# thangvubk/SoftGroup

Hardware: AMD Instinct MI355X
Metric: scans/sec ScanNet-v2-like inference (softgroup_scannet.yaml, full forward_test) (higher is better)
Workload: dtype f32

## Files before the change

### softgroup_amd/csrc/spconv_conv.hip

```cpp
#include <stdlib.h>

#include <atomic>
#include <cstdio>
#include <map>
#include <mutex>
#include <utility>
#include <vector>

#include "common.h"

namespace sg {

typedef float f32x16 __attribute__((ext_vector_type(16)));
typedef float f4 __attribute__((ext_vector_type(4)));
typedef float f2 __attribute__((ext_vector_type(2)));
typedef __bf16 bf16x8 __attribute__((ext_vector_type(8)));
typedef __bf16 bf16x2 __attribute__((ext_vector_type(2)));

__device__ __forceinline__ void split3(const float (&x)[8], bf16x8 &h, bf16x8 &m, bf16x8 &l) {
#pragma unroll
  for (int j = 0; j < 4; ++j) {
    const f2 v = {x[2 * j], x[2 * j + 1]};
    const bf16x2 hh = __builtin_convertvector(v, bf16x2);
    const f2 r = v - __builtin_convertvector(hh, f2);
// ... 173 lines not shown
    int k2 = k, s2 = s + 1;
    if (s2 == n_slices) {
      s2 = 0;
      const uint32_t rest = mask & ~((2u << k) - 1u);
      k2 = rest ? __builtin_ctz(rest) : -1;
    }
    if (k2 >= 0) load_raw(k2, s2, a_nxt, b_nxt);
    __builtin_amdgcn_sched_barrier(0);
#pragma unroll
    for (int j = 0; j < 8; ++j)
#pragma unroll
      for (int n = 0; n < NBW; ++n)
        acc[n] = __builtin_amdgcn_mfma_f32_32x32x2f32(a_cur[j], b_cur[n][j], acc[n], 0, 0, 0);
    __builtin_amdgcn_sched_barrier(0);
    k = k2;
    s = s2;
  }

  const bool final_out = p.ksplit == 1;
  float *out = p.out + (final_out ? 0 : static_cast<long long>(ks) * p.M_out * p.Cout);
  const bool add_res = p.residual != nullptr && final_out;
  const bool post = p.post_scale != nullptr && final_out;
  const bool act = p.out_act != nullptr && final_out;
  float ps[NBW], pb[NBW], as[NBW], ab[NBW];
#pragma unroll
  for (int n = 0; n < NBW; ++n) {
    ps[n] = post ? p.post_scale[coff[n]] : 1.f;
    pb[n] = post ? p.post_shift[coff[n]] : 0.f;
    as[n] = act ? p.act_scale[coff[n]] : 1.f;
    ab[n] = act ? p.act_shift[coff[n]] : 0.f;
  }
#pragma unroll
  for (int reg = 0; reg < 16; ++reg) {
    const int r = (reg & 3) + 8 * (reg >> 2) + 4 * ahalf;
    const int row = __shfl(my_row, r, 64);
    if (row < 0) continue;
    const long long off = static_cast<long long>(row) * p.Cout + col;
#pragma unroll
    for (int n = 0; n < NBW; ++n) {
      if (n < nbw && col + n * 32 < p.Cout) {
        float v = acc[n][reg];
        if (add_res) v += p.residual[off + n * 32];
        if (post) v = fmaxf(fmaf(v, ps[n], pb[n]), 0.f);
        out[off + n * 32] = v;
        if (act) p.out_act[off + n * 32] = fmaxf(fmaf(v, as[n], ab[n]), 0.f);
      }
    }
  }
}

constexpr int kRowsAt = kTileRows * kMaxK, kMaskAt = kRowsAt + kTileRows;
constexpr int kMetaInts = kMaskAt + 4;

template <int CK, int DEPTH, int TRACE, int NBW, int SPLIT, int WV, int AT, int CHAIN, int R16 = 0>
__device__ __forceinline__ void conv_layer_body(const ConvArgs &p, unsigned in_bytes, unsigned w_bytes) {
  static_assert(!R16 || (SPLIT == 2 && AT), "bf16 rows: bf16-operand arithmetic, line-wise gather");
  constexpr int AUX = CHAIN ? 16 : 0;
  static_assert(!SPLIT || CK == 16 || AT, "split-precision path: 16-channel slices");
  static_assert(!AT || (SPLIT && CK == 32), "line-wise gather: split path, 32-channel items");
  static_assert(WV == 2 || WV == 4 || WV == 8 || WV == 16, "2, 4, 8 or 16 waves per workgroup");
  constexpr int RR = 16 / WV;
  constexpr int WV_SHIFT = WV == 2 ? 1 : WV == 4 ? 2 : WV == 8 ? 3 : 4;
  constexpr int HC = CK / 2;
  constexpr int NQ = HC / 4;
  extern __shared__ __attribute__((aligned(16))) char smem_raw[];
  const int wave = __builtin_amdgcn_readfirstlane(threadIdx.x >> 6), lane = threadIdx.x & 63;
  const int arow = lane & 31, ahalf = lane >> 5;
  float *red = reinterpret_cast<float *>(smem_raw);
  int32_t *meta_lds = reinterpret_cast<int32_t *>(red + WV * NBW * 16 * 64);

  const int G = gridDim.x;
  const int units_per_tile = p.col_units * p.ksplit;
  const int num_units = p.num_units;
  const int n_slices = R16 ? (p.Cin + 63) / 64 : p.Cin / CK;
  const int c8 = p.Cin / 8;
  const int tileK = kTileRows * p.K;
  const int nbr_base = arow * p.K;
  const bool final_out = p.ksplit == 1;
  const bool add_res = p.residual != nullptr && final_out;
  const bool post = p.post_scale != nullptr && final_out;
  const bool act = p.out_act != nullptr && final_out;
  const bool combine = p.done != nullptr && !final_out;
  const int num_tiles = (p.M_out + kTileRows - 1) / kTileRows;
  const unsigned out_bytes = static_cast<unsigned>(p.M_out) * p.Cout * 4u;
  const bool out16 = SPLIT == 2 && p.out16 != 0, res16 = SPLIT == 2 && p.res16 != 0;
  const unsigned fin_bytes = out16 ? out_bytes >> 1 : out_bytes;
  const unsigned res_bytes = res16 ? out_bytes >> 1 : out_bytes;

  const __amdgpu_buffer_rsrc_t rs_in =
      __builtin_amdgcn_make_buffer_rsrc(const_cast<float *>(p.in), 0, in_bytes, 0x00020000);
  const __amdgpu_buffer_rsrc_t rs_w =
      __builtin_amdgcn_make_buffer_rsrc(const_cast<float *>(p.w), 0, w_bytes, 0x00020000);
  const __amdgpu_buffer_rsrc_t rs_res = __builtin_amdgcn_make_buffer_rsrc(
      const_cast<float *>(add_res ? p.residual : p.in), 0, add_res ? res_bytes : 0u, 0x00020000);
  const __amdgpu_buffer_rsrc_t rs_out = __builtin_amdgcn_make_buffer_rsrc(
      p.out, 0, final_out ? fin_bytes : out_bytes * static_cast<unsigned>(p.ksplit), 0x00020000);
  const __amdgpu_buffer_rsrc_t rs_act = __builtin_amdgcn_make_buffer_rsrc(
      act ? p.out_act : p.out, 0, act ? fin_bytes : 0u, 0x00020000);
  const bool c_res = combine && p.residual != nullptr, c_act = combine && p.out_act != nullptr;
  const __amdgpu_buffer_rsrc_t rs_cres = __builtin_amdgcn_make_buffer_rsrc(
      const_cast<float *>(c_res ? p.residual : p.in), 0, c_res ? res_bytes : 0u, 0x00020000);
  const __amdgpu_buffer_rsrc_t rs_cout = __builtin_amdgcn_make_buffer_rsrc(
      combine ? p.out_final : p.out, 0, combine ? fin_bytes : 0u, 0x00020000);
  const __amdgpu_buffer_rsrc_t rs_cact = __builtin_amdgcn_make_buffer_rsrc(
      c_act ? p.out_act : p.out, 0, c_act ? fin_bytes : 0u, 0x00020000);
  auto ld_row = [&](const __amdgpu_buffer_rsrc_t &rs, unsigned off, int n, bool h16) -> float {
    if constexpr (SPLIT == 2) {
      if (h16)
        return bf16_f32(static_cast<uint16_t>(__builtin_amdgcn_raw_buffer_load_b16(rs, off >> 1, n * 64, AUX)));
// ... 19 lines not shown
    Unit d;
    int sub;
    if (u < full) {
      const int blk = udiv(u >> 3, p.magic_upt);
      const int i = u - blk * group;
      d.tile = blk * 8 + (i & 7);
      sub = i >> 3;
    } else {
      d.tile = udiv(u, p.magic_upt);
      sub = u - d.tile * units_per_tile;
    }
    d.ks = udiv(sub, p.magic_cu);
    d.cu = sub - d.ks * p.col_units;
    return d;
  };

  int32_t *ctl = meta_lds + 2 * kMetaInts;
  const unsigned meta_lds_addr = __builtin_amdgcn_readfirstlane(
      static_cast<unsigned>(reinterpret_cast<uintptr_t>(meta_lds)));
  auto dma_meta = [&](int tile, int buf) {
    const unsigned dst = meta_lds_addr + static_cast<unsigned>(buf * kMetaInts) * 4u;
    const int32_t *blk = p.nbr_tiles + static_cast<long long>(tile) * tileK;
#pragma unroll
    for (int q = 0; q < 4; ++q) {
      const int e = q * 256 + lane * 4;
      if (e < tileK) lds_dma_b128(blk + e, dst + q * 1024);
    }
    if (lane < kTileRows) lds_dma_b32(p.order + tile * kTileRows + lane, dst + kRowsAt * 4);
    if (lane == 0) lds_dma_b32(p.tile_mask + tile, dst + kMaskAt * 4);
  };
  (void)num_tiles;

  constexpr int NPL = SPLIT == 2 ? 1 : 3;
  constexpr int NB_ = R16 ? 4 : AT ? 2 * NPL : SPLIT ? NPL : NQ;
  struct Slice { f4 a[NQ]; f4 b[NBW][NB_]; int nsl; };
  const int plane_bytes = p.K * c8 * p.Cout * 16;
  const int planes_at = 2 * plane_bytes;
  struct Ctx {
    const int32_t *meta;
    uint32_t wg_mask;
    int col, ks, k, s, kp, sp, rem;
    int pair;
    int v_w;
    float ps[NBW], pb[NBW], as[NBW], ab[NBW];
    unsigned o_off[RR];
    bool col_ok;
  };

  Slice S[DEPTH];
  float resv[NBW][RR];

  f4 *tr_lds = reinterpret_cast<f4 *>(ctl + 4) + wave * 256;
  const unsigned row_pitch = static_cast<unsigned>(p.Cin) * 4u, lane_chunk = static_cast<unsigned>(lane & 7) * 16u;
  auto load = [&](const Ctx &c, int k, int s, Slice &S) {
    if constexpr (R16) {
#pragma unroll
      for (int q = 0; q < 4; ++q) {
        const unsigned src = static_cast<unsigned>(c.meta[(8 * q + (lane >> 3)) * p.K + k]);
        const unsigned v_a = __umul24(src, row_pitch >> 1) + lane_chunk;
        S.a[q] = __builtin_bit_cast(f4, __builtin_amdgcn_raw_buffer_load_b128(rs_in, v_a, s * 128, AUX));
      }
      const int s_w = planes_at + (k * c8 + s * 8) * p.Cout * 16;
      const int nsl = s * 64 + 64 <= p.Cin ? 4 : 2;
      S.nsl = nsl;
#pragma unroll
      for (int n = 0; n < NBW; ++n)
#pragma unroll
        for (int sl = 0; sl < 4; ++sl)
          S.b[n][sl] = __builtin_bit_cast(f4, __builtin_amdgcn_raw_buffer_load_b128(
                                                  rs_w, c.v_w + n * 512, s_w + (sl < nsl ? sl : sl - 2) * (2 * p.Cout * 16), 0));
      return;
    }
    if constexpr (AT) {
#pragma unroll
      for (int q = 0; q < 4; ++q) {
        unsigned src = static_cast<unsigned>(c.meta[(8 * q + (lane >> 3)) * p.K + k]);
        if (SG_WHATIF & 16) src = static_cast<unsigned>(c.pair * 32 + 8 * q + (lane >> 3)) % static_cast<unsigned>(p.M_out);
        const unsigned v_a = __umul24(src, row_pitch) + lane_chunk;
        S.a[q] = __builtin_bit_cast(f4, __builtin_amdgcn_raw_buffer_load_b128(rs_in, v_a, s * 128, AUX));
      }
      const int s_w = planes_at + (k * c8 + s * 4) * p.Cout * 16;
#pragma unroll
      for (int n = 0; n < NBW; ++n)
#pragma unroll
        for (int sl = 0; sl < 2; ++sl)
#pragma unroll
          for (int pl = 0; pl < NPL; ++pl) {
            if ((SG_WHATIF & 1) && pl > 0) { S.b[n][sl * NPL + pl] = S.b[n][sl * NPL]; continue; }
            S.b[n][sl * NPL + pl] = __builtin_bit_cast(f4, __builtin_amdgcn_raw_buffer_load_b128(
                                                             rs_w, c.v_w + n * 512,
                                                             s_w + sl * (2 * p.Cout * 16) + pl * plane_bytes, 0));
          }
      return;
    }
    const int src = c.meta[nbr_base + k];
    const unsigned v_a = src >= 0 ? static_cast<unsigned>(src * p.Cin + ahalf * HC) * 4u : kOob;
    const int s_a = s * (CK * 4);
#pragma unroll
    for (int q = 0; q < NQ; ++q)
      S.a[q] = __builtin_bit_cast(f4, __builtin_amdgcn_raw_buffer_load_b128(rs_in, v_a + q * 16, s_a, AUX));
    if constexpr (SPLIT) {
      const int s_w = planes_at + (k * c8 + s * 2) * p.Cout * 16;
#pragma unroll
      for (int n = 0; n < NBW; ++n)
#pragma unroll
        for (int pl = 0; pl < NPL; ++pl)
          S.b[n][pl] = __builtin_bit_cast(f4, __builtin_amdgcn_raw_buffer_load_b128(
                                                  rs_w, c.v_w + n * 512, s_w + pl * plane_bytes, 0));
    } else {
      const int s_w = (k * c8 + s * (CK / 8)) * p.Cout * 32;
#pragma unroll
      for (int n = 0; n < NBW; ++n)
#pragma unroll
        for (int q = 0; q < NQ; ++q)
          S.b[n][q] = __builtin_bit_cast(f4, __builtin_amdgcn_raw_buffer_load_b128(
                                                 rs_w, c.v_w + n * 1024 + (q & 1) * 16,
                                                 s_w + (q >> 1) * (p.Cout * 32), 0));
    }
  };

  auto advance = [&](const Ctx &c, int &k, int &s) {
    if (++s == n_slices) {
      s = 0;
      const uint32_t rest = c.wg_mask & ~((2u << k) - 1u);
      k = rest ? __builtin_ctz(rest) : k;
    }
  };

  auto setup = [&](const Unit &d, int buf, Ctx &c) {
    c.ks = d.ks;
    c.pair = d.tile * p.col_units + d.cu;
    c.meta = meta_lds + buf * kMetaInts;
    uint32_t m = static_cast<uint32_t>(c.meta[kMaskAt]);
    if (!final_out) {
      const int k_lo = d.ks * p.k_per_split, k_hi = min(p.K, k_lo + p.k_per_split);
      m &= ((1u << k_hi) - 1u) & ~((1u << k_lo) - 1u);
    }
    m = __builtin_amdgcn_readfirstlane(m);
    c.wg_mask = m;
    c.col = d.cu * (32 * NBW) + arow;
    c.col_ok = c.col < p.Cout;
    const int colc = min(c.col, p.Cout - 1);
    c.v_w = SPLIT ? (ahalf * p.Cout + colc) * 16 : (ahalf * (HC / 8) * p.Cout + colc) * 32;
    const int items = __builtin_popcount(m) * n_slices;
    const int per = (items + WV - 1) >> WV_SHIFT;
// ... 110 lines not shown
          }
          acc[n] = __builtin_amdgcn_mfma_f32_32x32x16_bf16(al, bh, acc[n], 0, 0, 0);
          acc[n] = __builtin_amdgcn_mfma_f32_32x32x16_bf16(am, bm, acc[n], 0, 0, 0);
          acc[n] = __builtin_amdgcn_mfma_f32_32x32x16_bf16(ah, bl, acc[n], 0, 0, 0);
          acc[n] = __builtin_amdgcn_mfma_f32_32x32x16_bf16(am, bh, acc[n], 0, 0, 0);
          acc[n] = __builtin_amdgcn_mfma_f32_32x32x16_bf16(ah, bm, acc[n], 0, 0, 0);
          acc[n] = __builtin_amdgcn_mfma_f32_32x32x16_bf16(ah, bh, acc[n], 0, 0, 0);
        }
      }
      return;
    }
    if constexpr (SPLIT) {
      const float af[8] = {S.a[0][0], S.a[0][1], S.a[0][2], S.a[0][3], S.a[1][0], S.a[1][1], S.a[1][2], S.a[1][3]};
      if constexpr (SPLIT == 2) {
        const bf16x8 ah = round_bf16(af);
#pragma unroll
        for (int n = 0; n < NBW; ++n)
          acc[n] = __builtin_amdgcn_mfma_f32_32x32x16_bf16(ah, __builtin_bit_cast(bf16x8, S.b[n][0]), acc[n], 0,
                                                           0, 0);
        return;
      }
      bf16x8 ah, am, al;
      split3(af, ah, am, al);
#pragma unroll
      for (int n = 0; n < NBW; ++n) {
        const bf16x8 bh = __builtin_bit_cast(bf16x8, S.b[n][0]);
        const bf16x8 bm = __builtin_bit_cast(bf16x8, S.b[n][1]);
        const bf16x8 bl = __builtin_bit_cast(bf16x8, S.b[n][2]);
        acc[n] = __builtin_amdgcn_mfma_f32_32x32x16_bf16(al, bh, acc[n], 0, 0, 0);
        acc[n] = __builtin_amdgcn_mfma_f32_32x32x16_bf16(am, bm, acc[n], 0, 0, 0);
        acc[n] = __builtin_amdgcn_mfma_f32_32x32x16_bf16(ah, bl, acc[n], 0, 0, 0);
        acc[n] = __builtin_amdgcn_mfma_f32_32x32x16_bf16(am, bh, acc[n], 0, 0, 0);
        acc[n] = __builtin_amdgcn_mfma_f32_32x32x16_bf16(ah, bm, acc[n], 0, 0, 0);
        acc[n] = __builtin_amdgcn_mfma_f32_32x32x16_bf16(ah, bh, acc[n], 0, 0, 0);
      }
      return;
    }
#pragma unroll
    for (int q = 0; q < NQ; ++q) {
      asm volatile("" : "+v"(S.a[q]));
#pragma unroll
      for (int n = 0; n < NBW; ++n) asm volatile("" : "+v"(S.b[n][q]));
    }
    __builtin_amdgcn_sched_barrier(0);
#pragma unroll
    for (int q = 0; q < NQ; ++q)
#pragma unroll
      for (int j = 0; j < 4; ++j)
#pragma unroll
        for (int n = 0; n < NBW; ++n)
          acc[n] = __builtin_amdgcn_mfma_f32_32x32x2f32(S.a[q][j], S.b[n][q][j], acc[n], 0, 0, 0);
  };

  unsigned long long stamp[8];
  auto mark = [&](int i) {
    if constexpr (TRACE) stamp[i] = __builtin_readcyclecounter();
  };

  const int xcd = blockIdx.x & 7;
  const int dyn0 = (p.dyn_rounds == 1 ? 1 : 2) * G;
  const bool draws = p.queue != nullptr && dyn0 < num_units;
  const bool draw_first = draws && p.dyn_rounds == 1;
  auto barrier = [] {
    asm volatile("s_waitcnt lgkmcnt(0)\n\ts_barrier" ::: "memory");
  };

  if (static_cast<int>(blockIdx.x) >= num_units) return;
  int round = 0, u = blockIdx.x, buf = 0;
  Unit du = decode(u);
  unsigned ticket = 0;
  bool drawing = true;
  if (wave == 0) {
    if (lane == 0 && draw_first)
      ticket = __hip_atomic_fetch_add(p.queue + xcd * kTicketStride, 1u, __ATOMIC_RELAXED, __HIP_MEMORY_SCOPE_AGENT);
    dma_meta(du.tile, 0);
    asm volatile("s_waitcnt vmcnt(0)" ::: "memory");
  }
  barrier();
  Ctx c;
  setup(du, 0, c);

  while (true) {
    mark(0);
    int un_w0 = -1;
    if (wave == 0) {
      if ((round == 0 && !draw_first) || !draws) {
        const int r = round + 1;
        const int b = static_cast<int>(blockIdx.x);
        const int rev = (G & 7) == 0 ? G - 8 - (b & ~7) + (b & 7) : G - 1 - b;
        un_w0 = r * G + ((__builtin_popcount(r) & 1) ? rev : b);
      } else if (drawing) {
        const unsigned t = __builtin_amdgcn_readfirstlane(ticket);
        un_w0 = dyn0 + static_cast<int>(t) * 8 + xcd;
      }
      if (un_w0 >= num_units || un_w0 < 0) {
        un_w0 = -1;
        drawing = false;
      }
      if (un_w0 >= 0) dma_meta(decode(un_w0).tile, buf ^ 1);
      if (lane == 0) ctl[buf ^ 1] = un_w0;
    }
#pragma unroll
    for (int n = 0; n < NBW; ++n)
#pragma unroll
      for (int r = 0; r < 16; ++r) acc[n][r] = 0.f;
    {
      int kp = c.kp, sp = c.sp, issued = DEPTH - 1;
      const int rem = c.rem;
      for (int g = rem / DEPTH; g > 0; --g) {
#pragma unroll
        for (int i = 0; i < DEPTH; ++i) {
          int k2 = kp, s2 = sp;
          advance(c, k2, s2);
          const bool more = issued < rem;
          kp = more ? k2 : kp;
          sp = more ? s2 : sp;
          ++issued;
          load(c, kp, sp, S[(i + DEPTH - 1) % DEPTH]);
          __builtin_amdgcn_sched_barrier(0);
          compute(S[i]);
          __builtin_amdgcn_sched_barrier(0);
        }
      }
      const int tail = rem % DEPTH;
#pragma unroll
      for (int i = 0; i < DEPTH - 1; ++i)
        if (i < tail) compute(S[i]);
    }
    if constexpr (TRACE) { asm volatile("" : "+v"(acc[0][0])); }
    mark(1);

    if (wave == 0) {
      asm volatile("s_waitcnt vmcnt(0)" ::: "memory");
      if (lane == 0 && draws)
        ticket = __hip_atomic_fetch_add(p.queue + xcd * kTicketStride, 1u, __ATOMIC_RELAXED,
                                        __HIP_MEMORY_SCOPE_AGENT);
    }

    barrier();
    mark(2);
#pragma unroll
    for (int n = 0; n < NBW; ++n)
#pragma unroll
      for (int reg = 0; reg < 16; ++reg) red[((wave * NBW + n) * 16 + reg) * 64 + lane] = acc[n][reg];
    barrier();
    mark(3);
    const int un = __builtin_amdgcn_readfirstlane(ctl[buf ^ 1]);
    const bool has_next = un >= 0;
    const Unit dn = decode(has_next ? un : u);

    float v[NBW][RR], va[NBW][RR];
    unsigned o_off[RR];
    {
      float part[NBW][RR][WV];
#pragma unroll
      for (int n = 0; n < NBW; ++n)
#pragma unroll
        for (int rr = 0; rr < RR; ++rr) {
          const int reg = wave * RR + rr;
// ... 79 lines not shown
          for (int j = 0; j < 4; ++j)
#pragma unroll
            for (int rr = 0; rr < RR; ++rr)
#pragma unroll
              for (int n = 0; n < NBW; ++n) t[n][rr] += q[j][n][rr];
        }
        for (; ks < p.ksplit; ++ks) {
          float q[NBW][RR];
#pragma unroll
          for (int rr = 0; rr < RR; ++rr)
#pragma unroll
            for (int n = 0; n < NBW; ++n) q[n][rr] = part(ks, rr, n);
#pragma unroll
          for (int rr = 0; rr < RR; ++rr)
#pragma unroll
            for (int n = 0; n < NBW; ++n) t[n][rr] += q[n][rr];
        }
        float res[NBW][RR];
#pragma unroll
        for (int rr = 0; rr < RR; ++rr)
#pragma unroll
          for (int n = 0; n < NBW; ++n)
            res[n][rr] = ld_row(rs_cres, o_off[rr], n, res16);
#pragma unroll
        for (int rr = 0; rr < RR; ++rr)
#pragma unroll
          for (int n = 0; n < NBW; ++n) {
            float x = t[n][rr] + res[n][rr];
            if (p.post_scale) x = fmaxf(fmaf(x, ps[n], pb[n]), 0.f);
            st_row(x, rs_cout, o_off[rr], 0u, n, out16);
            st_row(fmaxf(fmaf(x, as[n], ab[n]), 0.f), rs_cact, o_off[rr], 0u, n, out16);
          }
      }
    }
    mark(5);
    if constexpr (TRACE) {
      if (lane == 0 && p.trace && wave < kWavesPerWg) {
        unsigned long long *t = p.trace + (static_cast<long long>(u) * kWavesPerWg + wave) * 8;
        for (int i = 0; i < 6; ++i) t[i] = stamp[i];
        unsigned hw, xcc;
        asm volatile("s_getreg_b32 %0, hwreg(HW_REG_HW_ID)" : "=s"(hw));
        asm volatile("s_getreg_b32 %0, hwreg(HW_REG_XCC_ID)" : "=s"(xcc));
        t[6] = static_cast<unsigned long long>(blockIdx.x);
        t[7] = (static_cast<unsigned long long>(rem_done) << 48) | (static_cast<unsigned long long>(xcc & 0xf) << 32) | hw;
      }
    }
    if (!has_next) break;
    u = un;
    ++round;
    buf ^= 1;
  }
}

template <int CK, int DEPTH, int TRACE, int WPE, int NBW = 1, int SPLIT = 0, int WV = 4, int AT = 0, int R16 = 0>
__global__ void __launch_bounds__(64 * WV, WPE) gather_conv_persistent_kernel(ConvArgs p, unsigned in_bytes,
                                                                             unsigned w_bytes) {
  conv_layer_body<CK, DEPTH, TRACE, NBW, SPLIT, WV, AT, 0, R16>(p, in_bytes, w_bytes);
}

struct ChainStep {
  const float *in, *w, *post_scale, *post_shift, *residual, *act_scale, *act_shift;
  float *out_act;
  const int32_t *order;
  const uint32_t *tile_mask;
  const int32_t *nbr_tiles;
  float *out;
  unsigned *done;
  float *out_final;
  int M_out, K, Cin, Cout, col_units, ksplit, k_per_split, num_units;
  unsigned magic_upt, magic_cu, magic_nsl, in_bytes, w_bytes;
  int kind;
  int pad_[2];
};
constexpr int kChainMax = 22;
struct ChainArgs {
  ChainStep s[kChainMax];
  unsigned *bar;
  unsigned *abort_host;
  unsigned long long *trace;
  int n;
};
static_assert(sizeof(ChainArgs) <= 4096, "the step list must fit the kernel-argument segment");
constexpr int kChainWV = 8;
constexpr int kChainBarWords = 18 * 32;
constexpr unsigned long long kChainTimeout = 200000000ull;

__device__ __forceinline__ bool chain_barrier(unsigned *bar, unsigned epoch, unsigned *abort_host, int *flag_lds,
                                              unsigned long long *stamp) {
  asm volatile("s_waitcnt vmcnt(0)" ::: "memory");
  __syncthreads();
  if (threadIdx.x == 0) {
    if (stamp) stamp[2] = __builtin_amdgcn_s_memrealtime();
    const unsigned x = blockIdx.x & 7, nx = (gridDim.x + 7u - x) >> 3;
    int ok = 1;
    const unsigned old = __hip_atomic_fetch_add(bar + x * 32, 1u, __ATOMIC_RELAXED, __HIP_MEMORY_SCOPE_AGENT);
    if (old == nx * epoch - 1u) {
      const unsigned groups = gridDim.x < 8u ? gridDim.x : 8u;
      const unsigned o2 = __hip_atomic_fetch_add(bar + 8 * 32, 1u, __ATOMIC_RELAXED, __HIP_MEMORY_SCOPE_AGENT);
      if (o2 == groups * epoch - 1u)
        for (unsigned j = 0; j < groups; ++j)
          __hip_atomic_store(bar + (9 + j) * 32, epoch, __ATOMIC_RELAXED, __HIP_MEMORY_SCOPE_AGENT);
    }
    const unsigned long long t0 = __builtin_amdgcn_s_memrealtime();
    unsigned spins = 0;
    while (__hip_atomic_load(bar + (9 + x) * 32, __ATOMIC_RELAXED, __HIP_MEMORY_SCOPE_AGENT) < epoch) {
      __builtin_amdgcn_s_sleep(2);
      if ((++spins & 255u) == 0u) {
        if (__hip_atomic_load(bar + 17 * 32, __ATOMIC_RELAXED, __HIP_MEMORY_SCOPE_AGENT) != 0u) { ok = 0; break; }
        if (__builtin_amdgcn_s_memrealtime() - t0 > kChainTimeout) {
          __hip_atomic_store(bar + 17 * 32, 1u, __ATOMIC_RELAXED, __HIP_MEMORY_SCOPE_AGENT);
// ... 471 lines not shown
    const int rc = chain_flush();
    if (rc != SG_OK) return rc;
  }
  if (conv) {
    c.b16 = b16;
    c.arith_set = true;
  }
  c.args.s[c.args.n++] = st;
  if (counts) ++c.conv_steps;
  return SG_OK;
}

void conv_chain_begin(hipStream_t stream) {
  ChainRec &c = t_chain;
  c.mode = chain_enabled() ? 2 : 1;
  c.stream = stream;
  c.args.n = 0;
  c.conv_steps = 0;
  c.arith_set = false;
}
bool conv_chain_recording() { return t_chain.mode == 2; }
int conv_chain_end() {
  const int rc = t_chain.mode == 2 ? chain_flush() : SG_OK;
  t_chain.mode = 0;
  t_chain.args.n = 0;
  return rc;
}
void conv_chain_abort() {
  t_chain.mode = 0;
  t_chain.args.n = 0;
  t_chain.conv_steps = 0;
}
int conv_chain_concat(const float *a, const float *b, int64_t rows, int ca, int cb, const float *scale,
                      const float *shift, float *out, float *out_act) {
  ChainStep st = {};
  st.kind = 1;
  st.in = a; st.residual = b; st.act_scale = scale; st.act_shift = shift; st.out = out; st.out_act = out_act;
  st.M_out = static_cast<int>(rows); st.Cin = ca; st.Cout = cb;
  return chain_push(st, t_chain.b16, false);
}
int conv_chain_bn_relu(const float *x, const float *scale, const float *shift, int64_t rows, int c, float *out) {
  ChainStep st = {};
  st.kind = 2;
  st.in = x; st.post_scale = scale; st.post_shift = shift; st.out = out;
  st.M_out = static_cast<int>(rows); st.Cin = c; st.Cout = 0;
  return chain_push(st, t_chain.b16, false);
}

typedef void (*PersistentFn)(ConvArgs, unsigned, unsigned);
struct SplitVariant {
  PersistentFn fn, fn_trace;
  PersistentFn fn_b16;
  PersistentFn fn_r16;
  int nbw, wv, ck, at;
  size_t lds;
  int occ, occ_b16, occ_r16;
};
#ifndef SG_B16_DEPTH
#define SG_B16_DEPTH 2
#endif
#ifndef SG_B16_WPE_PLUS
#define SG_B16_WPE_PLUS 0
#endif
template <int CK, int WPE, int NBW, int WV, int AT>
constexpr PersistentFn r16_variant() {
  if constexpr (AT) return gather_conv_persistent_kernel<CK, SG_B16_DEPTH, 0, WPE + SG_B16_WPE_PLUS, NBW, 2, WV, 1, 1>;
  else return nullptr;
}
#define SG_SPLIT_VARIANT(CK, DEPTH, WPE, NBW, WV, AT)                                            \
  {gather_conv_persistent_kernel<CK, DEPTH, 0, WPE, NBW, 1, WV, AT>,                              \
   gather_conv_persistent_kernel<CK, DEPTH, 1, WPE, NBW, 1, WV, AT>,                              \
   gather_conv_persistent_kernel<CK, SG_B16_DEPTH, 0, WPE + SG_B16_WPE_PLUS, NBW, 2, WV, AT>,     \
   r16_variant<CK, WPE, NBW, WV, AT>(), NBW, WV, CK, AT, 0, 0, 0, 0}
constexpr int kSplitVariants = 9;
static SplitVariant g_split_variants[kSplitVariants] = {
    SG_SPLIT_VARIANT(32, 2, 2, 2, 2, 1),  SG_SPLIT_VARIANT(32, 2, 3, 1, 2, 1),
    SG_SPLIT_VARIANT(32, 2, 2, 2, 4, 1),  SG_SPLIT_VARIANT(32, 2, 3, 1, 4, 1), SG_SPLIT_VARIANT(32, 2, 1, 1, 8, 1),
    SG_SPLIT_VARIANT(16, 2, 3, 2, 4, 0),  SG_SPLIT_VARIANT(16, 2, 4, 1, 4, 0), SG_SPLIT_VARIANT(16, 2, 2, 1, 8, 0),
    SG_SPLIT_VARIANT(16, 2, 1, 1, 16, 0),
};

static int launch_persistent_split(ConvArgs a, int num_tiles, long long in_bytes, long long w_bytes,
                                   hipStream_t stream, bool b16, bool in16) {
  static int num_cu = 0;
  static std::once_flag once;
  std::call_once(once, [] {
    int dev = 0;
    hipGetDevice(&dev);
    hipDeviceGetAttribute(&num_cu, hipDeviceAttributeMultiprocessorCount, dev);
    if (num_cu <= 0) num_cu = 256;
    auto prepare = [](SplitVariant &v) {
      v.lds = static_cast<size_t>(v.wv) * v.nbw * 16 * 64 * sizeof(float) + 2 * kMetaInts * sizeof(int32_t) + 16 +
              (v.at ? static_cast<size_t>(v.wv) * 4096 : 0);
      int o = 0;
      hipOccupancyMaxActiveBlocksPerMultiprocessor(&o, v.fn, 64 * v.wv, v.lds);
      v.occ = o < 1 ? 1 : o;
      o = 0;
      hipOccupancyMaxActiveBlocksPerMultiprocessor(&o, v.fn_b16, 64 * v.wv, v.lds);
      v.occ_b16 = o < 1 ? 1 : o;
      o = 0;
      if (v.fn_r16) hipOccupancyMaxActiveBlocksPerMultiprocessor(&o, v.fn_r16, 64 * v.wv, v.lds);
      v.occ_r16 = o < 1 ? 1 : o;
    };
    for (SplitVariant &v : g_split_variants) prepare(v);
  });
  static const int nbw_env = getenv("SG_CONV_NBW") ? atoi(getenv("SG_CONV_NBW")) : 2;
  static const int wv_env = getenv("SG_CONV_WV") ? atoi(getenv("SG_CONV_WV")) : 0;
  static const float min_rounds = getenv("SG_CONV_ROUNDS") ? atof(getenv("SG_CONV_ROUNDS")) : 2.5f;
  static const int at_env = getenv("SG_CONV_AT") ? atoi(getenv("SG_CONV_AT")) : 1;
  const int NB = (a.Cout + 31) / 32;
  const unsigned long long row_bytes = (in16 ? 2ull : 4ull) * a.Cin;
  const unsigned absent_at = static_cast<unsigned>((0xFFFFFFull * row_bytes) & 0xFFFFFFFFull);
  const int use_at = ((at_env != 0 || in16) && a.Cin % 32 == 0 && in_bytes / static_cast<long long>(row_bytes) < (1LL << 24) - 1 &&
                      static_cast<long long>(absent_at) >= in_bytes) ? 1 : 0;
  if (in16 && (!use_at || !b16)) {
    set_error("sg_unet_forward(bf16 rows): a layer with %d input channels / %lld input bytes cannot take the line-wise bf16 gather",
              a.Cin, in_bytes);
    return SG_ERR_ARG;
  }
  int pick = -1;
  static const int w2_max = getenv("SG_CONV_W2_MAX") ? atoi(getenv("SG_CONV_W2_MAX")) : 108;
  static const int w2_nbw = getenv("SG_CONV_W2_NBW") ? atoi(getenv("SG_CONV_W2_NBW")) : 2;
  static const float w2_rounds = getenv("SG_CONV_W2_ROUNDS") ? atof(getenv("SG_CONV_W2_ROUNDS")) : 1.5f;
  const bool use_w2 = wv_env == 2 || (wv_env == 0 && a.K * (a.Cin / 32) <= w2_max);
  for (int i = 0; i < kSplitVariants; ++i) {
    const SplitVariant &v = g_split_variants[i];
    if (v.at != use_at) continue;
    if (v.wv == 2 && (!use_w2 || a.ksplit > 1 || v.nbw > w2_nbw)) continue;
    if (a.ksplit > 1) {
      if (v.nbw == 1 && v.wv == 4) { pick = i; break; }
      continue;
    }
    pick = i;
    if (v.nbw == 2 && (a.Cout % 64 != 0 || nbw_env < 2)) continue;
    if (wv_env && v.wv != wv_env) continue;
    const long long units = static_cast<long long>(num_tiles) * (NB / v.nbw);
    if (wv_env || units >= static_cast<long long>((v.wv == 2 ? w2_rounds : min_rounds) * num_cu * (in16 ? v.occ_r16 : b16 ? v.occ_b16 : v.occ))) {
      pick = i;
      break;
    }
  }
  const bool chain_layer = t_chain.mode != 0 && use_at != 0;
  if (chain_layer) {
    for (int i = 0; i < kSplitVariants; ++i)
      if (g_split_variants[i].at == 1 && g_split_variants[i].nbw == 1 && g_split_variants[i].wv == kChainWV) pick = i;
  }
  const SplitVariant &v = g_split_variants[pick];
  a.col_units = NB / v.nbw;
  a.blocks_per_unit = v.nbw;
  const long long units = static_cast<long long>(num_tiles) * a.col_units * a.ksplit;
  a.num_units = static_cast<int>(units);
  auto magic = [](unsigned d) { return d <= 1 ? 0u : static_cast<unsigned>((1ULL << 32) / d) + 1u; };
  a.magic_upt = magic(static_cast<unsigned>(a.col_units * a.ksplit));
  a.magic_cu = magic(static_cast<unsigned>(a.col_units));
  a.magic_nsl = magic(static_cast<unsigned>(in16 ? (a.Cin + 63) / 64 : a.Cin / v.ck));
  if (t_chain.mode == 2) {
    if (chain_layer && !in16 && !a.out16 && !a.res16 && (a.ksplit == 1 || a.done != nullptr) && stream == t_chain.stream) {
      ChainStep st = {};
      st.kind = 0;
      st.in = a.in; st.w = a.w; st.post_scale = a.post_scale; st.post_shift = a.post_shift; st.residual = a.residual;
      st.act_scale = a.act_scale; st.act_shift = a.act_shift; st.out_act = a.out_act; st.order = a.order;
      st.tile_mask = a.tile_mask; st.nbr_tiles = a.nbr_tiles; st.out = a.out; st.done = a.done; st.out_final = a.out_final;
      st.M_out = a.M_out; st.K = a.K; st.Cin = a.Cin; st.Cout = a.Cout; st.col_units = a.col_units;
      st.ksplit = a.ksplit; st.k_per_split = a.k_per_split; st.num_units = a.num_units;
      st.magic_upt = a.magic_upt; st.magic_cu = a.magic_cu; st.magic_nsl = a.magic_nsl;
      st.in_bytes = static_cast<unsigned>(in_bytes); st.w_bytes = static_cast<unsigned>(w_bytes);
      return chain_push(st, b16, a.K > 1);
    }
    const int rc = chain_flush();
    if (rc != SG_OK) return rc;
  }
  static const bool dyn_env = getenv("SG_CONV_STATIC") && atoi(getenv("SG_CONV_STATIC")) == 0;
  static const int dyn_rounds_env = getenv("SG_CONV_DYN_ROUNDS") ? atoi(getenv("SG_CONV_DYN_ROUNDS")) : 2;
  a.queue = dyn_env ? take_tickets(stream) : nullptr;
  a.dyn_rounds = dyn_rounds_env == 1 ? 1 : 2;
  long long g = static_cast<long long>(num_cu) * (in16 ? v.occ_r16 : b16 ? v.occ_b16 : v.occ);
  if (g >= 8) g -= g % 8;
  if (units < g) g = units >= 8 ? (units + 7) / 8 * 8 : units;
  const unsigned ib = static_cast<unsigned>(in_bytes), wb = static_cast<unsigned>(w_bytes);
  if (in16) {
    v.fn_r16<<<static_cast<int>(g), 64 * v.wv, v.lds, stream>>>(a, ib, wb);
    return check_launch("sg_spconv_gather_conv(bf16 rows)");
  }
  if (b16) {
    v.fn_b16<<<static_cast<int>(g), 64 * v.wv, v.lds, stream>>>(a, ib, wb);
    return check_launch("sg_spconv_gather_conv_f32(bf16 operands)");
  }
  static const char *trace_env = getenv("SG_CONV_TRACE");
  if (trace_env) {
    const size_t nb = static_cast<size_t>(units) * kWavesPerWg * 8 * sizeof(unsigned long long);
    unsigned long long *dbuf = nullptr;
    hipMalloc(&dbuf, nb);
    hipMemsetAsync(dbuf, 0, nb, stream);
    a.trace = dbuf;
    v.fn_trace<<<static_cast<int>(g), 64 * v.wv, v.lds, stream>>>(a, ib, wb);
    hipStreamSynchronize(stream);
    std::vector<unsigned long long> h(nb / 8);
    hipMemcpy(h.data(), dbuf, nb, hipMemcpyDeviceToHost);
    hipFree(dbuf);
    if (FILE *f = fopen(trace_env, "ab")) {
      long long hdr[8] = {a.M_out, a.K, a.Cin, a.Cout, units, a.col_units, v.wv, g};
      fwrite(hdr, 8, 8, f);
      fwrite(h.data(), 8, h.size(), f);
      fclose(f);
    }
  } else {
    v.fn<<<static_cast<int>(g), 64 * v.wv, v.lds, stream>>>(a, ib, wb);
  }
  return check_launch("sg_spconv_gather_conv_f32(split)");
}


}

using namespace sg;

extern "C" {

int sg_spconv_set_arithmetic(int mode) {
  SG_REQUIRE(mode >= -1 && mode <= 2, "sg_spconv_set_arithmetic: mode must be -1, 0, 1 or 2");
  g_arith_override = mode;
  return SG_OK;
}

int sg_spconv_set_combine(int mode) {
  SG_REQUIRE(mode >= -1 && mode <= 1, "sg_spconv_set_combine: mode must be -1, 0 or 1");
  g_combine_override = mode;
  return SG_OK;
}

int sg_spconv_set_chain(int mode) {
  SG_REQUIRE(mode >= -1 && mode <= 1, "sg_spconv_set_chain: mode must be -1, 0 or 1");
  g_chain_override = mode;
  return SG_OK;
}

int sg_spconv_chain_stats(int64_t *launches, int64_t *steps) {
  if (launches) *launches = g_chain_launches.load(std::memory_order_relaxed);
  if (steps) *steps = g_chain_steps.load(std::memory_order_relaxed);
  return SG_OK;
}

int sg_spconv_profile(int enable) {
  g_conv_prof.enabled = enable != 0;
  if (enable) {
    g_conv_prof.used = 0;
    g_conv_prof.dims.clear();
  }
  return SG_OK;
}

int sg_spconv_profile_detail(float *ms, int32_t *dims, int cap, int *calls) {
  const int n = static_cast<int>(g_conv_prof.used / 2);
  if (calls) *calls = n;
  for (int i = 0; i < n && i < cap; ++i) {
    if (hipEventSynchronize(g_conv_prof.pool[2 * i + 1]) != hipSuccess) {
      set_error("sg_spconv_profile_detail: event synchronisation failed");
      return SG_ERR_LAUNCH;
    }
    float t = 0.f;
// ... 248 lines not shown
```

Measured before the change: 402.8.

## Add software-pipelined two-stage item loop for split-precision line-wise conv

Adds a PIPE template variant of the split-precision line-wise gather conv. Each item is processed in two halves: the LDS transpose, fragment read and bf16 three-way split for the next half are interleaved with the MFMA chain of the current half, and row loads for the next item are issued early. sched_group_barrier hints set the MFMA/VALU/DS interleaving. The variant is selected for full-kernel (K==kMaxK), Cin>=64, non-split, non-chain f32 layers on variants enabled by a compile-time mask. This raises register pressure and may lower occupancy.

```diff
diff --git a/softgroup_amd/csrc/spconv_conv.hip b/softgroup_amd/csrc/spconv_conv.hip
--- a/softgroup_amd/csrc/spconv_conv.hip
+++ b/softgroup_amd/csrc/spconv_conv.hip
@@ -249,9 +249,11 @@
 constexpr int kRowsAt = kTileRows * kMaxK, kMaskAt = kRowsAt + kTileRows;
 constexpr int kMetaInts = kMaskAt + 4;
 
-template <int CK, int DEPTH, int TRACE, int NBW, int SPLIT, int WV, int AT, int CHAIN, int R16 = 0>
+template <int CK, int DEPTH, int TRACE, int NBW, int SPLIT, int WV, int AT, int CHAIN, int R16 = 0, int PIPE = 0>
 __device__ __forceinline__ void conv_layer_body(const ConvArgs &p, unsigned in_bytes, unsigned w_bytes) {
   static_assert(!R16 || (SPLIT == 2 && AT), "bf16 rows: bf16-operand arithmetic, line-wise gather");
+  static_assert(!PIPE || (SPLIT == 1 && AT && !R16 && !CHAIN && DEPTH == 2),
+                "two-stage item loop: split-precision line-wise path, two ring slots");
   constexpr int AUX = CHAIN ? 16 : 0;
   static_assert(!SPLIT || CK == 16 || AT, "split-precision path: 16-channel slices");
   static_assert(!AT || (SPLIT && CK == 32), "line-wise gather: split path, 32-channel items");
@@ -377,26 +379,8 @@
 
   f4 *tr_lds = reinterpret_cast<f4 *>(ctl + 4) + wave * 256;
   const unsigned row_pitch = static_cast<unsigned>(p.Cin) * 4u, lane_chunk = static_cast<unsigned>(lane & 7) * 16u;
-  auto load = [&](const Ctx &c, int k, int s, Slice &S) {
-    if constexpr (R16) {
-#pragma unroll
-      for (int q = 0; q < 4; ++q) {
-        const unsigned src = static_cast<unsigned>(c.meta[(8 * q + (lane >> 3)) * p.K + k]);
-        const unsigned v_a = __umul24(src, row_pitch >> 1) + lane_chunk;
-        S.a[q] = __builtin_bit_cast(f4, __builtin_amdgcn_raw_buffer_load_b128(rs_in, v_a, s * 128, AUX));
-      }
-      const int s_w = planes_at + (k * c8 + s * 8) * p.Cout * 16;
-      const int nsl = s * 64 + 64 <= p.Cin ? 4 : 2;
-      S.nsl = nsl;
-#pragma unroll
-      for (int n = 0; n < NBW; ++n)
-#pragma unroll
-        for (int sl = 0; sl < 4; ++sl)
-          S.b[n][sl] = __builtin_bit_cast(f4, __builtin_amdgcn_raw_buffer_load_b128(
-                                                  rs_w, c.v_w + n * 512, s_w + (sl < nsl ? sl : sl - 2) * (2 * p.Cout * 16), 0));
-      return;
-    }
-    if constexpr (AT) {
+  auto load_a = [&](const Ctx &c, int k, int s, Slice &S) {
+    if constexpr (AT && !R16) {
 #pragma unroll
       for (int q = 0; q < 4; ++q) {
         unsigned src = static_cast<unsigned>(c.meta[(8 * q + (lane >> 3)) * p.K + k]);
@@ -404,6 +388,10 @@
         const unsigned v_a = __umul24(src, row_pitch) + lane_chunk;
         S.a[q] = __builtin_bit_cast(f4, __builtin_amdgcn_raw_buffer_load_b128(rs_in, v_a, s * 128, AUX));
       }
+    }
+  };
+  auto load_b = [&](const Ctx &c, int k, int s, Slice &S) {
+    if constexpr (AT && !R16) {
       const int s_w = planes_at + (k * c8 + s * 4) * p.Cout * 16;
 #pragma unroll
       for (int n = 0; n < NBW; ++n)
@@ -416,6 +404,30 @@
                                                              rs_w, c.v_w + n * 512,
                                                              s_w + sl * (2 * p.Cout * 16) + pl * plane_bytes, 0));
           }
+    }
+  };
+  auto load = [&](const Ctx &c, int k, int s, Slice &S) {
+    if constexpr (R16) {
+#pragma unroll
+      for (int q = 0; q < 4; ++q) {
+        const unsigned src = static_cast<unsigned>(c.meta[(8 * q + (lane >> 3)) * p.K + k]);
+        const unsigned v_a = __umul24(src, row_pitch >> 1) + lane_chunk;
+        S.a[q] = __builtin_bit_cast(f4, __builtin_amdgcn_raw_buffer_load_b128(rs_in, v_a, s * 128, AUX));
+      }
+      const int s_w = planes_at + (k * c8 + s * 8) * p.Cout * 16;
+      const int nsl = s * 64 + 64 <= p.Cin ? 4 : 2;
+      S.nsl = nsl;
+#pragma unroll
+      for (int n = 0; n < NBW; ++n)
+#pragma unroll
+        for (int sl = 0; sl < 4; ++sl)
+          S.b[n][sl] = __builtin_bit_cast(f4, __builtin_amdgcn_raw_buffer_load_b128(
+                                                  rs_w, c.v_w + n * 512, s_w + (sl < nsl ? sl : sl - 2) * (2 * p.Cout * 16), 0));
+      return;
+    }
+    if constexpr (AT) {
+      load_a(c, k, s, S);
+      load_b(c, k, s, S);
       return;
     }
     const int src = c.meta[nbr_base + k];
@@ -632,6 +644,39 @@
           acc[n] = __builtin_amdgcn_mfma_f32_32x32x2f32(S.a[q][j], S.b[n][q][j], acc[n], 0, 0, 0);
   };
 
+  constexpr int kPipeMfma = 12 * NBW;
+  struct Half { bf16x8 h, m, l; };
+  auto rows_to_lds = [&](const Slice &S) {
+#pragma unroll
+    for (int q = 0; q < 4; ++q) {
+      const int r = 8 * q + (lane >> 3);
+      tr_lds[r * 8 + ((lane & 7) ^ ((r >> 1) & 7))] = S.a[q];
+    }
+  };
+  auto read_frag = [&](int sl, f4 (&fr)[2]) {
+#pragma unroll
+    for (int j = 0; j < 2; ++j) fr[j] = tr_lds[arow * 8 + ((sl * 4 + ahalf * 2 + j) ^ ((arow >> 1) & 7))];
+  };
+  auto split_half = [&](const f4 (&fr)[2], Half &H) {
+    const float af[8] = {fr[0][0], fr[0][1], fr[0][2], fr[0][3], fr[1][0], fr[1][1], fr[1][2], fr[1][3]};
+    split3(af, H.h, H.m, H.l);
+  };
+  auto mma_half = [&](const Half &H, const Slice &S, int sl) {
+#pragma unroll
+    for (int n = 0; n < NBW; ++n) {
+      const bf16x8 bh = __builtin_bit_cast(bf16x8, S.b[n][sl * 3 + 0]);
+      const bf16x8 bm = __builtin_bit_cast(bf16x8, S.b[n][sl * 3 + 1]);
+      const bf16x8 bl = __builtin_bit_cast(bf16x8, S.b[n][sl * 3 + 2]);
+      acc[n] = __builtin_amdgcn_mfma_f32_32x32x16_bf16(H.l, bh, acc[n], 0, 0, 0);
+      acc[n] = __builtin_amdgcn_mfma_f32_32x32x16_bf16(H.m, bm, acc[n], 0, 0, 0);
+      acc[n] = __builtin_amdgcn_mfma_f32_32x32x16_bf16(H.h, bl, acc[n], 0, 0, 0);
+      acc[n] = __builtin_amdgcn_mfma_f32_32x32x16_bf16(H.m, bh, acc[n], 0, 0, 0);
+      acc[n] = __builtin_amdgcn_mfma_f32_32x32x16_bf16(H.h, bm, acc[n], 0, 0, 0);
+      acc[n] = __builtin_amdgcn_mfma_f32_32x32x16_bf16(H.h, bh, acc[n], 0, 0, 0);
+    }
+  };
+  constexpr int kHalfValu = (44 + kPipeMfma / 2 - 2) / (kPipeMfma / 2 - 1);
+
   unsigned long long stamp[8];
   auto mark = [&](int i) {
     if constexpr (TRACE) stamp[i] = __builtin_readcyclecounter();
@@ -684,7 +729,81 @@
     for (int n = 0; n < NBW; ++n)
 #pragma unroll
       for (int r = 0; r < 16; ++r) acc[n][r] = 0.f;
-    {
+    if constexpr (PIPE) {
+      int ka = c.kp, sa = c.sp, next_rows = 1;
+      const int rem = c.rem;
+      auto request_rows = [&](Slice &Sx) {
+        int k2 = ka, s2 = sa;
+        advance(c, k2, s2);
+        const bool more = next_rows < rem;
+        ka = more ? k2 : ka;
+        sa = more ? s2 : sa;
+        ++next_rows;
+        load_a(c, ka, sa, Sx);
+      };
+      Half H0;
+      {
+        f4 f0[2];
+        rows_to_lds(S[0]);
+        request_rows(S[0]);
+        read_frag(0, f0);
+        __builtin_amdgcn_sched_barrier(0);
+        split_half(f0, H0);
+        __builtin_amdgcn_sched_barrier(0);
+      }
+      auto interleave = [](int ds_at) {
+        __builtin_amdgcn_sched_group_barrier(0x008, 1, 0);
+        if (ds_at == 1) __builtin_amdgcn_sched_group_barrier(0x100, 2, 0);
+#pragma unroll
+        for (int i = 0; i < kPipeMfma / 2 - 1; ++i) {
+          __builtin_amdgcn_sched_group_barrier(0x008, 1, 0);
+          if (ds_at == i + 2) __builtin_amdgcn_sched_group_barrier(0x100, 2, 0);
+          __builtin_amdgcn_sched_group_barrier(0x002, kHalfValu, 0);
+        }
+      };
+      auto trip = [&](const Slice &cur, Slice &nxt, bool request) {
+        f4 f1[2], f0[2];
+        Half H1, Hn;
+        read_frag(1, f1);
+        rows_to_lds(S[0]);
+        load_b(c, ka, sa, nxt);
+        if (request) request_rows(S[0]);
+        __builtin_amdgcn_sched_barrier(0);
+        read_frag(0, f0);
+        split_half(f1, H1);
+        mma_half(H0, cur, 0);
+        interleave(NBW == 1 ? 1 : 7);
+        __builtin_amdgcn_sched_barrier(0);
+        split_half(f0, Hn);
+        mma_half(H1, cur, 1);
+        interleave(0);
+        __builtin_amdgcn_sched_barrier(0);
+        H0 = Hn;
+      };
+      auto last = [&](const Slice &cur) {
+        f4 f1[2];
+        Half H1;
+        read_frag(1, f1);
+        __builtin_amdgcn_sched_barrier(0);
+        split_half(f1, H1);
+        mma_half(H0, cur, 0);
+        interleave(0);
+        __builtin_amdgcn_sched_barrier(0);
+        mma_half(H1, cur, 1);
+        __builtin_amdgcn_sched_barrier(0);
+      };
+      const int steady = rem - 1;
+      for (int g = steady >> 1; g > 0; --g) {
+        trip(S[0], S[1], true);
+        trip(S[1], S[0], true);
+      }
+      if (steady > 0 && (steady & 1)) {
+        trip(S[0], S[1], false);
+        last(S[1]);
+      } else if (rem > 0) {
+        last(S[0]);
+      }
+    } else {
       int kp = c.kp, sp = c.sp, issued = DEPTH - 1;
       const int rem = c.rem;
       for (int g = rem / DEPTH; g > 0; --g) {
@@ -870,10 +989,10 @@
   }
 }
 
-template <int CK, int DEPTH, int TRACE, int WPE, int NBW = 1, int SPLIT = 0, int WV = 4, int AT = 0, int R16 = 0>
+template <int CK, int DEPTH, int TRACE, int WPE, int NBW = 1, int SPLIT = 0, int WV = 4, int AT = 0, int R16 = 0, int PIPE = 0>
 __global__ void __launch_bounds__(64 * WV, WPE) gather_conv_persistent_kernel(ConvArgs p, unsigned in_bytes,
                                                                              unsigned w_bytes) {
-  conv_layer_body<CK, DEPTH, TRACE, NBW, SPLIT, WV, AT, 0, R16>(p, in_bytes, w_bytes);
+  conv_layer_body<CK, DEPTH, TRACE, NBW, SPLIT, WV, AT, 0, R16, PIPE>(p, in_bytes, w_bytes);
 }
 
 struct ChainStep {
@@ -1451,10 +1570,20 @@
   PersistentFn fn, fn_trace;
   PersistentFn fn_b16;
   PersistentFn fn_r16;
+  PersistentFn fn_pipe, fn_pipe_trace;
   int nbw, wv, ck, at;
   size_t lds;
-  int occ, occ_b16, occ_r16;
+  int occ, occ_b16, occ_r16, occ_pipe;
 };
+#ifndef SG_CONV_PIPE_MASK
+#define SG_CONV_PIPE_MASK 0x1b
+#endif
+template <int CK, int WPE, int NBW, int WV, int AT, int TRACE, int ON>
+constexpr PersistentFn pipe_variant() {
+  if constexpr (AT && ON) return gather_conv_persistent_kernel<CK, 2, TRACE, WPE, NBW, 1, WV, 1, 0, 1>;
+  else return nullptr;
+}
+#define SG_PIPE_OF(i) (SG_CONV_PIPE_MASK >> (i) & 1)
 #ifndef SG_B16_DEPTH
 #define SG_B16_DEPTH 2
 #endif
@@ -1466,17 +1595,19 @@
   if constexpr (AT) return gather_conv_persistent_kernel<CK, SG_B16_DEPTH, 0, WPE + SG_B16_WPE_PLUS, NBW, 2, WV, 1, 1>;
   else return nullptr;
 }
-#define SG_SPLIT_VARIANT(CK, DEPTH, WPE, NBW, WV, AT)                                            \
+#define SG_SPLIT_VARIANT(CK, DEPTH, WPE, NBW, WV, AT, PIPE)                                      \
   {gather_conv_persistent_kernel<CK, DEPTH, 0, WPE, NBW, 1, WV, AT>,                              \
    gather_conv_persistent_kernel<CK, DEPTH, 1, WPE, NBW, 1, WV, AT>,                              \
    gather_conv_persistent_kernel<CK, SG_B16_DEPTH, 0, WPE + SG_B16_WPE_PLUS, NBW, 2, WV, AT>,     \
-   r16_variant<CK, WPE, NBW, WV, AT>(), NBW, WV, CK, AT, 0, 0, 0, 0}
+   r16_variant<CK, WPE, NBW, WV, AT>(), pipe_variant<CK, WPE, NBW, WV, AT, 0, (PIPE)>(),          \
+   pipe_variant<CK, WPE, NBW, WV, AT, 1, (PIPE)>(), NBW, WV, CK, AT, 0, 0, 0, 0, 0}
 constexpr int kSplitVariants = 9;
 static SplitVariant g_split_variants[kSplitVariants] = {
-    SG_SPLIT_VARIANT(32, 2, 2, 2, 2, 1),  SG_SPLIT_VARIANT(32, 2, 3, 1, 2, 1),
-    SG_SPLIT_VARIANT(32, 2, 2, 2, 4, 1),  SG_SPLIT_VARIANT(32, 2, 3, 1, 4, 1), SG_SPLIT_VARIANT(32, 2, 1, 1, 8, 1),
-    SG_SPLIT_VARIANT(16, 2, 3, 2, 4, 0),  SG_SPLIT_VARIANT(16, 2, 4, 1, 4, 0), SG_SPLIT_VARIANT(16, 2, 2, 1, 8, 0),
-    SG_SPLIT_VARIANT(16, 2, 1, 1, 16, 0),
+    SG_SPLIT_VARIANT(32, 2, 2, 2, 2, 1, SG_PIPE_OF(0)),       SG_SPLIT_VARIANT(32, 2, 3, 1, 2, 1, SG_PIPE_OF(1)),
+    SG_SPLIT_VARIANT(32, 2, 2, 2, 4, 1, SG_PIPE_OF(2)),  SG_SPLIT_VARIANT(32, 2, 3, 1, 4, 1, SG_PIPE_OF(3)),
+    SG_SPLIT_VARIANT(32, 2, 1, 1, 8, 1, SG_PIPE_OF(4)),
+    SG_SPLIT_VARIANT(16, 2, 3, 2, 4, 0, 0),  SG_SPLIT_VARIANT(16, 2, 4, 1, 4, 0, 0), SG_SPLIT_VARIANT(16, 2, 2, 1, 8, 0, 0),
+    SG_SPLIT_VARIANT(16, 2, 1, 1, 16, 0, 0),
 };
 
 static int launch_persistent_split(ConvArgs a, int num_tiles, long long in_bytes, long long w_bytes,
@@ -1500,6 +1631,9 @@
       o = 0;
       if (v.fn_r16) hipOccupancyMaxActiveBlocksPerMultiprocessor(&o, v.fn_r16, 64 * v.wv, v.lds);
       v.occ_r16 = o < 1 ? 1 : o;
+      o = 0;
+      if (v.fn_pipe) hipOccupancyMaxActiveBlocksPerMultiprocessor(&o, v.fn_pipe, 64 * v.wv, v.lds);
+      v.occ_pipe = o < 1 ? 1 : o;
     };
     for (SplitVariant &v : g_split_variants) prepare(v);
   });
@@ -1573,7 +1707,8 @@
   static const int dyn_rounds_env = getenv("SG_CONV_DYN_ROUNDS") ? atoi(getenv("SG_CONV_DYN_ROUNDS")) : 2;
   a.queue = dyn_env ? take_tickets(stream) : nullptr;
   a.dyn_rounds = dyn_rounds_env == 1 ? 1 : 2;
-  long long g = static_cast<long long>(num_cu) * (in16 ? v.occ_r16 : b16 ? v.occ_b16 : v.occ);
+  const bool pipe = v.fn_pipe != nullptr && !b16 && !in16 && a.K == kMaxK && a.Cin >= 64 && a.ksplit == 1 && !chain_layer;
+  long long g = static_cast<long long>(num_cu) * (in16 ? v.occ_r16 : b16 ? v.occ_b16 : pipe ? v.occ_pipe : v.occ);
   if (g >= 8) g -= g % 8;
   if (units < g) g = units >= 8 ? (units + 7) / 8 * 8 : units;
   const unsigned ib = static_cast<unsigned>(in_bytes), wb = static_cast<unsigned>(w_bytes);
@@ -1592,7 +1727,7 @@
     hipMalloc(&dbuf, nb);
     hipMemsetAsync(dbuf, 0, nb, stream);
     a.trace = dbuf;
-    v.fn_trace<<<static_cast<int>(g), 64 * v.wv, v.lds, stream>>>(a, ib, wb);
+    (pipe ? v.fn_pipe_trace : v.fn_trace)<<<static_cast<int>(g), 64 * v.wv, v.lds, stream>>>(a, ib, wb);
     hipStreamSynchronize(stream);
     std::vector<unsigned long long> h(nb / 8);
     hipMemcpy(h.data(), dbuf, nb, hipMemcpyDeviceToHost);
@@ -1604,7 +1739,7 @@
       fclose(f);
     }
   } else {
-    v.fn<<<static_cast<int>(g), 64 * v.wv, v.lds, stream>>>(a, ib, wb);
+    (pipe ? v.fn_pipe : v.fn)<<<static_cast<int>(g), 64 * v.wv, v.lds, stream>>>(a, ib, wb);
   }
   return check_launch("sg_spconv_gather_conv_f32(split)");
 }
```

Result: slower. 391.4 (-2.8%).
